# 0xMiden/miden-vm

Hardware: AMD Instinct MI355X
Metric: trace rows/sec proved (2^20-row trace, 96-bit sec) (higher is better)
Workload: dtype u64 (Goldilocks field, p = 2^64 - 2^32 + 1); 1 GPU; full proof of miden:20:51:8 (DummyMidenAir 2^20 x 51 + 8 EF aux), 96-bit production PCS params (blowup 8, FRI arity 4, 27 queries, PoW 4/12/16), Poseidon2 LMCS; trace resident in HBM, transcript on host; log_trace_rows=20, main_width=51, aux_width_ef=8, log_blowup=3, proof_bytes=137697, parallelism=1 GPU

## Files before the change

miden-vm_amd/csrc/deep.hip:

```cpp
#include "gl.cuh"
#include "kernels.hpp"

__global__ __launch_bounds__(256) void k_bary_weights(const u64* tw, int log_n, u64 g, e2 y0, e2 y1, u64* w0, u64* w1) {
  const size_t n = (size_t)1 << log_n;
  const size_t base = (size_t)blockIdx.x * 1024 + threadIdx.x;
  const size_t half = n >> 1;
  u64 xs[4], nrm[8], pre[8];
  e2 den[8];
#pragma unroll
  for (int k = 0; k < 4; k++) {
    size_t r = base + (size_t)k * 256;
    u64 x = 0;
    if (r < n) x = gl_mul(g, half ? (r < half ? tw[r] : gl_neg(tw[r - half])) : 1);
    xs[k] = x;
    den[2 * k] = e2_sub(y0, e2_make(x));
    den[2 * k + 1] = e2_sub(y1, e2_make(x));
  }
  u64 run = 1;
#pragma unroll
  for (int k = 0; k < 8; k++) {
    nrm[k] = gl_sub(gl_sqr(den[k].c0), gl_mul7(gl_sqr(den[k].c1)));
    pre[k] = run;
    run = gl_mul(run, nrm[k]);
  }
  u64 inv = gl_inv(run);
#pragma unroll
  for (int k = 7; k >= 0; k--) {
    u64 ni = gl_mul(inv, pre[k]);
    inv = gl_mul(inv, nrm[k]);
    size_t r = base + (size_t)(k >> 1) * 256;
    if (r < n) {
      u64 s = gl_mul(ni, xs[k >> 1]);
      u64* w = (k & 1) ? w1 : w0;
      w[2 * r] = gl_mul(den[k].c0, s);
      w[2 * r + 1] = gl_mul(gl_neg(den[k].c1), s);
    }
  }
}

static constexpr int OOD_ROWS_PER_BLOCK = 8192;
__global__ __launch_bounds__(256) void k_ood_partial(const u64* lde, int log_n, int log_blowup, const u64* w0, const u64* w1,
                                                     u64* partial, unsigned chunks) {
  __shared__ u64 red[4][256];
  const size_t n = (size_t)1 << log_n;
  const size_t col = blockIdx.y, chunk = blockIdx.x;
  const u64* f = lde + ((col << log_blowup) << log_n);
  const size_t r0 = chunk * OOD_ROWS_PER_BLOCK;
  const size_t r1 = r0 + OOD_ROWS_PER_BLOCK < n ? r0 + OOD_ROWS_PER_BLOCK : n;
  e2 a0 = e2_make(0), a1 = e2_make(0);
  for (size_t r = r0 + threadIdx.x; r < r1; r += 256) {
    u64 v = f[r];
    a0 = e2_add(a0, e2_mulf(e2{w0[2 * r], w0[2 * r + 1]}, v));
    a1 = e2_add(a1, e2_mulf(e2{w1[2 * r], w1[2 * r + 1]}, v));
  }
  red[0][threadIdx.x] = a0.c0; red[1][threadIdx.x] = a0.c1; red[2][threadIdx.x] = a1.c0; red[3][threadIdx.x] = a1.c1;
  __syncthreads();
  for (int s = 128; s > 0; s >>= 1) {
    if ((int)threadIdx.x < s) {
#pragma unroll
      for (int k = 0; k < 4; k++) red[k][threadIdx.x] = gl_add(red[k][threadIdx.x], red[k][threadIdx.x + s]);
    }
    __syncthreads();
  }
  if (threadIdx.x < 4) partial[(col * chunks + chunk) * 4 + threadIdx.x] = red[threadIdx.x][0];
}

void deep_ood_eval_batch(mh_ctx* c, std::vector<OodJob>& jobs, int log_blowup) {
  struct Weights {
    int log_n;
    size_t coset0;
    e2 y0, y1;
    DevBuf w0, w1;
  };
  std::vector<std::unique_ptr<Weights>> weights;
  struct Slot {
    size_t off = 0, ncol = 0;
    unsigned chunks = 0;
  };
  std::vector<Slot> slots(jobs.size());
  size_t total = 0;
  for (size_t k = 0; k < jobs.size(); k++) {
    OodJob& j = jobs[k];
    const LdeMatrix& m = *j.m;
    if (j.col_end > m.width) j.col_end = m.width;
    j.out0.assign(m.width, e2_make(0));
    j.out1.assign(m.width, e2_make(0));
    if (j.col_begin >= j.col_end) continue;
    const size_t n = (size_t)1 << m.log_n;
    slots[k].ncol = j.col_end - j.col_begin;
    slots[k].chunks = (unsigned)((n + OOD_ROWS_PER_BLOCK - 1) / OOD_ROWS_PER_BLOCK);
    slots[k].off = total;
    total += slots[k].ncol * slots[k].chunks * 4;
  }
  if (!total) return;
  DevBuf partial(total * 8), one;
  for (size_t k = 0; k < jobs.size(); k++) {
    if (!slots[k].ncol) continue;
    const OodJob& j = jobs[k];
    const LdeMatrix& m = *j.m;
    const int log_n = m.log_n;
    const size_t n = (size_t)1 << log_n;
    const u64 g = gl_mul(gl_lde_shift(log_n + log_blowup), gl_pow(gl_two_adic_generator(log_n + log_blowup), m.coset0));
    const u64* tw = log_n ? c->twiddles(log_n, false) : nullptr;
    if (!tw) {
      if (!one.p) {
        one.alloc(8);
        u64 v = 1;
        c->h2d(one.p, &v, 8);
      }
      tw = one.u();
    }
    ProfScope ps(c, "deep_ood_eval", (double)n * 8.0 * slots[k].ncol + 64.0 * n);
    Weights* w = nullptr;
    for (auto& cand : weights)
      if (cand->log_n == log_n && cand->coset0 == m.coset0 && e2_eq(cand->y0, j.y0) && e2_eq(cand->y1, j.y1)) w = cand.get();
    if (!w) {
      weights.emplace_back(new Weights{log_n, m.coset0, j.y0, j.y1, DevBuf(n * 16), DevBuf(n * 16)});
      w = weights.back().get();
      MH_LAUNCH(k_bary_weights, dim3((unsigned)((n + 1023) / 1024)), dim3(256), 0, c->stream, tw, log_n, g, j.y0, j.y1, w->w0.u(), w->w1.u());
    }
    MH_LAUNCH(k_ood_partial, dim3(slots[k].chunks, (unsigned)slots[k].ncol), dim3(256), 0, c->stream,
              m.lde.u() + ((j.col_begin << m.log_cosets) << log_n), log_n, m.log_cosets, w->w0.u(), w->w1.u(), partial.u() + slots[k].off,
              slots[k].chunks);
  }
  std::vector<u64> host(total);
  c->d2h(host.data(), partial.p, total * 8);
  for (size_t k = 0; k < jobs.size(); k++) {
    if (!slots[k].ncol) continue;
    OodJob& j = jobs[k];
    const LdeMatrix& m = *j.m;
    const int log_n = m.log_n;
    const size_t n = (size_t)1 << log_n;
    const u64 g = gl_mul(gl_lde_shift(log_n + log_blowup), gl_pow(gl_two_adic_generator(log_n + log_blowup), m.coset0));
    const u64 g_inv = gl_inv(g), n_inv = gl_inv((u64)n % GL_P);
    const e2 s0 = e2_mulf(e2_sub(e2_exp_pow2(e2_mulf(j.y0, g_inv), log_n), e2_make(1)), n_inv);
    const e2 s1 = e2_mulf(e2_sub(e2_exp_pow2(e2_mulf(j.y1, g_inv), log_n), e2_make(1)), n_inv);
    for (size_t col = 0; col < slots[k].ncol; col++) {
      e2 a0 = e2_make(0), a1 = e2_make(0);
      for (unsigned ch = 0; ch < slots[k].chunks; ch++) {
        const u64* p = host.data() + slots[k].off + (col * slots[k].chunks + ch) * 4;
        a0 = e2_add(a0, e2{p[0], p[1]});
        a1 = e2_add(a1, e2{p[2], p[3]});
      }
      j.out0[j.col_begin + col] = e2_mul(a0, s0);
      j.out1[j.col_begin + col] = e2_mul(a1, s1);
    }
  }
}
void deep_ood_eval_matrix(mh_ctx* c, const LdeMatrix& m, int log_blowup, e2 y0, e2 y1, std::vector<e2>& out0, std::vector<e2>& out1,
                          size_t col_begin, size_t col_end) {
  std::vector<OodJob> jobs(1);
  jobs[0].m = &m; jobs[0].y0 = y0; jobs[0].y1 = y1; jobs[0].col_begin = col_begin; jobs[0].col_end = col_end;
  deep_ood_eval_batch(c, jobs, log_blowup);
  out0.swap(jobs[0].out0);
  out1.swap(jobs[0].out1);
}

static constexpr int DEEP_MAX_MATS = 128;
static constexpr unsigned DEEP_FLUSH = 128;
#ifndef DEEP_UNROLL
#define DEEP_UNROLL 2
#endif
#ifndef DEEP_PTS_N
#define DEEP_PTS_N 1
#endif
static constexpr int DEEP_PTS = DEEP_PTS_N;
struct DeepMat {
  const u64* lde;
  u32 width, coef_off;
  int log_n;
};
struct DeepArgs {
  DeepMat m[DEEP_MAX_MATS];
  int n_mats, log_n, log_blowup;
  const u64* negc;
  const u64* tw;
  const u64* coset_x;
  e2 z0, z1, fred0, fred1, beta;
  u64* out;
};

__global__ __launch_bounds__(256) void k_deep_assemble(DeepArgs a) {
  const size_t N = (size_t)1 << a.log_n;
  const size_t j = blockIdx.y;
  const size_t base = (size_t)blockIdx.x * (256 * DEEP_PTS) + threadIdx.x;
  size_t r[DEEP_PTS];
#pragma unroll
  for (int k = 0; k < DEEP_PTS; k++) r[k] = base + (size_t)k * 256;
  e2 neg[DEEP_PTS];
  u64 w[DEEP_PTS][2][6];
#pragma unroll
  for (int k = 0; k < DEEP_PTS; k++) {
    neg[k] = e2_make(0);
#pragma unroll
    for (int e = 0; e < 2; e++)
#pragma unroll
      for (int i = 0; i < 6; i++) w[k][e][i] = 0;
  }
  auto flush = [&]() {
    const u64 C[6] = {1ULL, 1ULL << 22, 1ULL << 44, 1ULL << 32, 1ULL << 54, GL_EPS << 12};
#pragma unroll
    for (int k = 0; k < DEEP_PTS; k++) {
      u64 s0 = w[k][0][0], s1 = w[k][1][0];
#pragma unroll
      for (int i = 1; i < 6; i++) {
        s0 = gl_add(s0, gl_mul(w[k][0][i], C[i]));
        s1 = gl_add(s1, gl_mul(w[k][1][i], C[i]));
      }
      neg[k] = e2_add(neg[k], e2{s0, s1});
#pragma unroll
      for (int e = 0; e < 2; e++)
#pragma unroll
        for (int i = 0; i < 6; i++) w[k][e][i] = 0;
    }
  };
  u32 pending = 0;
#pragma unroll 1
  for (int mi = 0; mi < a.n_mats; mi++) {
    const DeepMat m = a.m[mi];
    const size_t nm_mask = ((size_t)1 << m.log_n) - 1;
    const u64* colp = m.lde + (j << m.log_n);
    const size_t cstride = (size_t)1 << (m.log_n + a.log_blowup);
#pragma unroll DEEP_UNROLL
    for (u32 cidx = 0; cidx < m.width; cidx++) {
      const u64 cf0 = a.negc[2 * (m.coef_off + cidx)], cf1 = a.negc[2 * (m.coef_off + cidx) + 1];
      u32 al[2][3];
#pragma unroll
      for (int i = 0; i < 3; i++) {
        al[0][i] = (u32)(cf0 >> (22 * i)) & 0x3FFFFFu;
        al[1][i] = (u32)(cf1 >> (22 * i)) & 0x3FFFFFu;
      }
#pragma unroll
      for (int k = 0; k < DEEP_PTS; k++) {
        if (r[k] < N) {
          const u64 v = colp[r[k] & nm_mask];
          const u32 v0 = (u32)v, v1 = (u32)(v >> 32);
#pragma unroll
          for (int e = 0; e < 2; e++) {
            w[k][e][0] += (u64)al[e][0] * v0;
            w[k][e][1] += (u64)al[e][1] * v0;
            w[k][e][2] += (u64)al[e][2] * v0;
            w[k][e][3] += (u64)al[e][0] * v1;
            w[k][e][4] += (u64)al[e][1] * v1;
            w[k][e][5] += (u64)al[e][2] * v1;
          }
        }
      }
      colp += cstride;
      if (++pending == DEEP_FLUSH) {
        flush();
        pending = 0;
      }
    }
  }
  flush();
  const size_t half = N >> 1;
  const u64 cx = a.coset_x[j];
  e2 den[2 * DEEP_PTS];
  u64 nrm[2 * DEEP_PTS], pre[2 * DEEP_PTS];
#pragma unroll
  for (int k = 0; k < DEEP_PTS; k++) {
    u64 x = 0;
    if (r[k] < N) x = gl_mul(cx, half ? (r[k] < half ? a.tw[r[k]] : gl_neg(a.tw[r[k] - half])) : 1);
    den[2 * k] = e2_sub(a.z0, e2_make(x));
    den[2 * k + 1] = e2_sub(a.z1, e2_make(x));
  }
  u64 run = 1;
#pragma unroll
  for (int k = 0; k < 2 * DEEP_PTS; k++) {
    nrm[k] = gl_sub(gl_sqr(den[k].c0), gl_mul7(gl_sqr(den[k].c1)));
    pre[k] = run;
    run = gl_mul(run, nrm[k]);
  }
  u64 inv = gl_inv(run);
  e2 qinv[2 * DEEP_PTS];
#pragma unroll
  for (int k = 2 * DEEP_PTS - 1; k >= 0; k--) {
    u64 ni = gl_mul(inv, pre[k]);
    inv = gl_mul(inv, nrm[k]);
    qinv[k] = e2{gl_mul(den[k].c0, ni), gl_mul(gl_neg(den[k].c1), ni)};
  }
#pragma unroll
  for (int k = 0; k < DEEP_PTS; k++) {
    if (r[k] < N) {
      e2 v = e2_mul(qinv[2 * k], e2_add(a.fred0, neg[k]));
      v = e2_add(v, e2_mul(e2_mul(a.beta, qinv[2 * k + 1]), e2_add(a.fred1, neg[k])));
      ulonglong2* o = reinterpret_cast<ulonglong2*>(a.out + 2 * ((j << a.log_n) + r[k]));
      *o = make_ulonglong2(v.c0, v.c1);
    }
  }
}

void deep_assemble(mh_ctx* c, const std::vector<const LdeMatrix*>& mats, const std::vector<u32>& coef_off, int log_n, int log_blowup,
                   const std::vector<e2>& negc, e2 z0, e2 z1, e2 fred0, e2 fred1, e2 beta, u64* out) {
  MH_REQUIRE(mats.size() <= (size_t)DEEP_MAX_MATS, "too many committed matrices for one DEEP pass");
  const int lbl = mats[0]->log_cosets;
  const size_t coset0 = mats[0]->coset0;
  for (auto* m : mats) MH_REQUIRE(m->log_cosets == lbl && m->coset0 == coset0, "internal: matrices cover different cosets");
  const size_t N = (size_t)1 << log_n, B = (size_t)1 << lbl;
  const int L = log_n + log_blowup;
  std::vector<u64> blob;
  for (e2 v : negc) { blob.push_back(v.c0); blob.push_back(v.c1); }
  const size_t o_cx = blob.size();
  const u64 g = gl_lde_shift(L), wK = gl_two_adic_generator(L);
  u64 x = gl_mul(g, gl_pow(wK, coset0));
  for (size_t j = 0; j < B; j++) {
    blob.push_back(x);
    x = gl_mul(x, wK);
  }
  DevBuf dblob(blob.size() * 8), one;
  c->h2d(dblob.p, blob.data(), blob.size() * 8);
  const u64* tw = log_n ? c->twiddles(log_n, false) : nullptr;
  if (!tw) {
    one.alloc(8);
    u64 v = 1;
    c->h2d(one.p, &v, 8);
    tw = one.u();
  }
  DeepArgs a{};
  double bytes = 16.0 * N * B;
  for (size_t i = 0; i < mats.size(); i++) {
    a.m[i] = DeepMat{mats[i]->lde.u(), (u32)mats[i]->width, coef_off[i], mats[i]->log_n};
    bytes += 8.0 * (double)mats[i]->width * (double)(((size_t)1 << mats[i]->log_n) << lbl);
  }
  a.n_mats = (int)mats.size();
  a.log_n = log_n; a.log_blowup = lbl;
  a.negc = dblob.u(); a.tw = tw; a.coset_x = dblob.u() + o_cx;
  a.z0 = z0; a.z1 = z1; a.fred0 = fred0; a.fred1 = fred1; a.beta = beta; a.out = out;
  {
    ProfScope ps(c, "deep_assemble", bytes);
    MH_LAUNCH(k_deep_assemble, dim3((unsigned)((N + 256 * DEEP_PTS - 1) / (256 * DEEP_PTS)), (unsigned)B), dim3(256), 0, c->stream, a);
  }
  HIP_CHECK(hipStreamSynchronize(c->stream));
}
```

miden-vm_amd/csrc/fri.hip:

```cpp
#include <cstring>
#include "gl.cuh"
#include "../../include/midenhip.h"
#include "kernels.hpp"
#include "blake3.cuh"
#include "keccak.cuh"
#include "poseidon2_fast.cuh"
#define RESCUE_FAST 1
#include "rescue.cuh"

__device__ __forceinline__ e2 ld_e2(const u64* p, size_t idx) {
  const ulonglong2 v = *reinterpret_cast<const ulonglong2*>(p + 2 * idx);
  return e2{v.x, v.y};
}
__device__ __forceinline__ void st_e2(u64* p, size_t idx, e2 v) { *reinterpret_cast<ulonglong2*>(p + 2 * idx) = make_ulonglong2(v.c0, v.c1); }

__device__ __forceinline__ u32 fri_row_pos(u32 p, int log_arity) { return bitrev32(p, log_arity); }

__global__ __launch_bounds__(256) void k_fri_leaf_hash(const u64* __restrict__ ev, int log_rows , int cbits, int log_arity,
                                                       u64* __restrict__ digests) {
  const int log_q = log_rows - log_arity;
  const size_t leaves = (size_t)1 << (log_q + cbits);
  const size_t s = blockIdx.x * (size_t)256 + threadIdx.x;
  if (s >= leaves) return;
  const size_t j = s >> log_q, r0 = s & (((size_t)1 << log_q) - 1);
  const u32 arity = 1u << log_arity;
  u64 st[12];
#pragma unroll
  for (int i = 0; i < 12; i++) st[i] = 0;
  for (u32 p0 = 0; p0 < arity; p0 += 4) {
#pragma unroll
    for (u32 k = 0; k < 4; k++) {
      e2 v = e2_make(0);
      if (p0 + k < arity) v = ld_e2(ev, (j << log_rows) + r0 + ((size_t)fri_row_pos(p0 + k, log_arity) << log_q));
      st[2 * k] = (p0 + k < arity) ? v.c0 : 0;
      st[2 * k + 1] = (p0 + k < arity) ? v.c1 : 0;
    }
    p2f_permute(st);
  }
  ulonglong2* o = reinterpret_cast<ulonglong2*>(digests + 4 * s);
  o[0] = make_ulonglong2(st[0], st[1]);
  o[1] = make_ulonglong2(st[2], st[3]);
}

__global__ __launch_bounds__(256) void k_fri_leaf_hash_b3(const u64* __restrict__ ev, int log_rows, int cbits, int log_arity,
                                                          u64* __restrict__ digests) {
  const int log_q = log_rows - log_arity;
  const size_t leaves = (size_t)1 << (log_q + cbits);
  const size_t s = blockIdx.x * (size_t)256 + threadIdx.x;
  if (s >= leaves) return;
  const size_t j = s >> log_q, r0 = s & (((size_t)1 << log_q) - 1);
  const u32 arity = 1u << log_arity;
  const u32 total = 32 + 16 * arity, n_blocks = (total + 63) / 64;
  b3::Stream h;
  h.init();
  uint32_t m[16], out[8];
#pragma unroll 1
  for (u32 b = 0; b < n_blocks; b++) {
    const int p0 = (int)(4 * b) - 2;
#pragma unroll
    for (int k = 0; k < 4; k++) {
      const int pp = p0 + k;
      e2 v = e2_make(0);
      if (pp >= 0 && (u32)pp < arity) v = ld_e2(ev, (j << log_rows) + r0 + ((size_t)fri_row_pos((u32)pp, log_arity) << log_q));
      m[4 * k] = (uint32_t)v.c0; m[4 * k + 1] = (uint32_t)(v.c0 >> 32);
      m[4 * k + 2] = (uint32_t)v.c1; m[4 * k + 3] = (uint32_t)(v.c1 >> 32);
    }
    if (b + 1 < n_blocks) h.block(m);
    else h.finish(m, total - 64 * b, out);
  }
#pragma unroll
  for (int i = 0; i < 4; i++) digests[4 * s + i] = (u64)out[2 * i] | ((u64)out[2 * i + 1] << 32);
}

__global__ __launch_bounds__(256) void k_fri_leaf_hash_alg(const u64* __restrict__ ev, int log_rows, int cbits, int log_arity,
                                                           u64* __restrict__ digests, int lmcs) {
  const int log_q = log_rows - log_arity;
  const size_t leaves = (size_t)1 << (log_q + cbits);
  const size_t s = blockIdx.x * (size_t)256 + threadIdx.x;
  if (s >= leaves) return;
  const size_t j = s >> log_q, r0 = s & (((size_t)1 << log_q) - 1);
  const u32 arity = 1u << log_arity;
  u64 st[12];
#pragma unroll
  for (int i = 0; i < 12; i++) st[i] = 0;
#pragma unroll 1
  for (u32 p0 = 0; p0 < arity; p0 += 4) {
#pragma unroll
    for (u32 k = 0; k < 4; k++) {
      e2 v = e2_make(0);
      if (p0 + k < arity) v = ld_e2(ev, (j << log_rows) + r0 + ((size_t)fri_row_pos(p0 + k, log_arity) << log_q));
      st[2 * k] = (p0 + k < arity) ? v.c0 : 0;
      st[2 * k + 1] = (p0 + k < arity) ? v.c1 : 0;
    }
    alg_permute(lmcs, st);
  }
#pragma unroll
  for (int i = 0; i < 4; i++) digests[4 * s + i] = st[i];
}

__global__ __launch_bounds__(256) void k_fri_leaf_hash_kk(const u64* __restrict__ ev, int log_rows, int cbits, int log_arity,
                                                          u64* __restrict__ digests) {
  const int log_q = log_rows - log_arity;
  const size_t leaves = (size_t)1 << (log_q + cbits);
  const size_t s = blockIdx.x * (size_t)256 + threadIdx.x;
  if (s >= leaves) return;
  const size_t j = s >> log_q, r0 = s & (((size_t)1 << log_q) - 1);
  const u32 arity = 1u << log_arity;
  uint64_t st[25];
#pragma unroll
  for (int i = 0; i < 25; i++) st[i] = 0;
#pragma unroll
  for (u32 p = 0; p < 8; p++) {
    if (p < arity) {
      const e2 v = ld_e2(ev, (j << log_rows) + r0 + ((size_t)fri_row_pos(p, log_arity) << log_q));
      st[2 * p] = v.c0;
      st[2 * p + 1] = v.c1;
    }
  }
  kk::f1600(st);
#pragma unroll
  for (int i = 0; i < 4; i++) digests[4 * s + i] = st[i];
}

struct FoldArgs {
  const u64* ev;
  u64* out;
  int log_rows, cbits, log_arity;
  const u64* tw_inv;
  const u64* coset_inv;
  e2 beta;
  u64 w4, w8_inv, inv_arity;
};
__global__ __launch_bounds__(256) void k_fri_fold(FoldArgs a) {
  const int log_q = a.log_rows - a.log_arity;
  const size_t total = (size_t)1 << (log_q + a.cbits);
  const size_t s = blockIdx.x * (size_t)256 + threadIdx.x;
  if (s >= total) return;
  const size_t j = s >> log_q, r0 = s & (((size_t)1 << log_q) - 1);
  const u64 s_inv = gl_mul(a.log_rows ? a.tw_inv[r0] : 1, a.coset_inv[j]);
  const e2 x = e2_mulf(a.beta, s_inv);
  const size_t base = (j << a.log_rows) + r0;
  e2 res;
  if (a.log_arity == 1) {
    e2 y0 = ld_e2(a.ev, base), y1 = ld_e2(a.ev, base + ((size_t)1 << log_q));
    res = e2_add(e2_add(y0, y1), e2_mul(e2_sub(y0, y1), x));
  } else if (a.log_arity == 3) {
    e2 y[8];
#pragma unroll
    for (int m = 0; m < 8; m++) y[m] = ld_e2(a.ev, base + ((size_t)m << log_q));
    const u64 wi1 = a.w8_inv, wi2 = gl_mul(wi1, wi1), wi3 = gl_mul(wi2, wi1);
#pragma unroll
    for (int m = 0; m < 4; m++) {
      const e2 u = y[m], v = y[m + 4];
      y[m] = e2_add(u, v);
      const e2 d = e2_sub(u, v);
      y[m + 4] = m == 0 ? d : e2_mulf(d, m == 1 ? wi1 : (m == 2 ? wi2 : wi3));
    }
#pragma unroll
    for (int h = 0; h < 8; h += 4)
#pragma unroll
      for (int m = 0; m < 2; m++) {
        const e2 u = y[h + m], v = y[h + m + 2];
        y[h + m] = e2_add(u, v);
        const e2 d = e2_sub(u, v);
        y[h + m + 2] = m == 0 ? d : e2_mulf(d, wi2);
      }
#pragma unroll
    for (int h = 0; h < 8; h += 2) {
      const e2 u = y[h], v = y[h + 1];
      y[h] = e2_add(u, v);
      y[h + 1] = e2_sub(u, v);
    }
    res = y[7];
    res = e2_add(e2_mul(res, x), y[3]);
    res = e2_add(e2_mul(res, x), y[5]);
    res = e2_add(e2_mul(res, x), y[1]);
    res = e2_add(e2_mul(res, x), y[6]);
    res = e2_add(e2_mul(res, x), y[2]);
    res = e2_add(e2_mul(res, x), y[4]);
    res = e2_add(e2_mul(res, x), y[0]);
  } else {
    e2 y0 = ld_e2(a.ev, base), y1 = ld_e2(a.ev, base + ((size_t)1 << log_q)), y2 = ld_e2(a.ev, base + ((size_t)2 << log_q)),
       y3 = ld_e2(a.ev, base + ((size_t)3 << log_q));
    e2 s02 = e2_add(y0, y2), d02 = e2_sub(y0, y2), s13 = e2_add(y1, y3), d31w = e2_mulf(e2_sub(y3, y1), a.w4);
    e2 c0 = e2_add(s02, s13), c1 = e2_add(d02, d31w), c2 = e2_sub(s02, s13), c3 = e2_sub(d02, d31w);
    e2 x2 = e2_sqr(x), x3 = e2_mul(x2, x);
    res = e2_add(e2_add(c0, e2_mul(c1, x)), e2_add(e2_mul(c2, x2), e2_mul(c3, x3)));
  }
  st_e2(a.out, s, e2_mulf(res, a.inv_arity));
}

__global__ void k_fri_to_natural(const u64* ev, u64* out, int log_rows, int cbits) {
  const size_t total = (size_t)1 << (log_rows + cbits);
  const size_t i = blockIdx.x * (size_t)blockDim.x + threadIdx.x;
  if (i >= total) return;
  const size_t j = i & (((size_t)1 << cbits) - 1), r = i >> cbits;
  st_e2(out, i, ld_e2(ev, (j << log_rows) + r));
}

void fri_leaf_hash(mh_ctx* c, const u64* ev, int log_rows, int cbits, int log_arity, u64* digests) {
  const size_t leaves = (size_t)1 << (log_rows - log_arity + cbits);
  ProfScope ps(c, "fri_leaf_hash", (double)leaves * (16.0 * (1 << log_arity) + 32.0));
  if (c->lmcs == MH_LMCS_RPO || c->lmcs == MH_LMCS_RPX)
    MH_LAUNCH(k_fri_leaf_hash_alg, dim3((unsigned)((leaves + 255) / 256)), dim3(256), 0, c->stream, ev, log_rows, cbits, log_arity, digests,
                       c->lmcs);
  else if (c->lmcs == MH_LMCS_KECCAK)
    MH_LAUNCH(k_fri_leaf_hash_kk, dim3((unsigned)((leaves + 255) / 256)), dim3(256), 0, c->stream, ev, log_rows, cbits, log_arity, digests);
  else if (c->lmcs == MH_LMCS_BLAKE3)
    MH_LAUNCH(k_fri_leaf_hash_b3, dim3((unsigned)((leaves + 255) / 256)), dim3(256), 0, c->stream, ev, log_rows, cbits, log_arity, digests);
  else
    MH_LAUNCH(k_fri_leaf_hash, dim3((unsigned)((leaves + 255) / 256)), dim3(256), 0, c->stream, ev, log_rows, cbits, log_arity,
                       digests);
}

void fri_fold(mh_ctx* c, const u64* ev, int log_rows, int cbits, int cbits_global, size_t coset0, int log_arity, e2 beta, u64* out) {
  MH_REQUIRE(log_arity >= 1 && log_arity <= 3, "FRI folding arity must be 2, 4 or 8");
  MH_REQUIRE(log_rows >= log_arity, "internal: FRI layer too short for a coset-major fold");
  const int logn = log_rows + cbits_global;
  const size_t C = (size_t)1 << cbits;
  std::vector<u64> ci(C);
  const u64 wn_inv = gl_inv(gl_two_adic_generator(logn));
  u64 x = gl_pow(wn_inv, coset0);
  for (size_t j = 0; j < C; j++) {
    ci[j] = x;
    x = gl_mul(x, wn_inv);
  }
  DevBuf d(C * 8);
  c->h2d(d.p, ci.data(), C * 8);
  FoldArgs a{};
  a.ev = ev; a.out = out; a.log_rows = log_rows; a.cbits = cbits; a.log_arity = log_arity;
  a.tw_inv = log_rows ? c->twiddles(log_rows, true) : nullptr;
  a.coset_inv = d.u();
  a.beta = beta;
  a.w4 = gl_two_adic_generator(2);
  a.w8_inv = gl_inv(gl_two_adic_generator(3));
  a.inv_arity = gl_inv((u64)1 << log_arity);
  const size_t total = (size_t)1 << (log_rows + cbits - log_arity);
  {
    ProfScope ps(c, "fri_fold", (double)total * 16.0 * ((1 << log_arity) + 1));
    MH_LAUNCH(k_fri_fold, dim3((unsigned)((total + 255) / 256)), dim3(256), 0, c->stream, a);
  }
  HIP_CHECK(hipStreamSynchronize(c->stream));
}

void fri_to_natural(mh_ctx* c, const u64* ev, int log_rows, int cbits, u64* out) {
  const size_t total = (size_t)1 << (log_rows + cbits);
  MH_LAUNCH(k_fri_to_natural, dim3((unsigned)((total + 255) / 256)), dim3(256), 0, c->stream, ev, out, log_rows, cbits);
}

struct GrindArgs {
  u64 st[12];
  u64 in[8];
  int n_in, bits;
  u64 base;
  unsigned long long* best;
};
__global__ __launch_bounds__(256) void k_grind(GrindArgs a) {
  const u64 w = a.base + blockIdx.x * (u64)256 + threadIdx.x;
  if (w >= GL_P) return;
  u64 s[12];
#pragma unroll
  for (int i = 0; i < 12; i++) s[i] = a.st[i];
  const int k = a.n_in + 1;
#pragma unroll
  for (int i = 0; i < 8; i++) {
    u64 v = (i < a.n_in) ? a.in[i] : (i == a.n_in ? w : 0);
    s[i] = (i < k) ? v : 0;
  }
  s[8] = gl_add(s[8], (u64)k);
  p2f_permute(s);
  const u64 x = s[7];
  if (((x & 0xFFFFFFFFULL) & (((u64)1 << a.bits) - 1)) == 0) atomicMin(a.best, (unsigned long long)w);
}

__global__ __launch_bounds__(256) void k_grind_alg(GrindArgs a, int lmcs) {
  const u64 w = a.base + blockIdx.x * (u64)256 + threadIdx.x;
  if (w >= GL_P) return;
  u64 s[12];
#pragma unroll
  for (int i = 0; i < 12; i++) s[i] = a.st[i];
  const int k = a.n_in + 1;
#pragma unroll
  for (int i = 0; i < 8; i++) {
    u64 v = (i < a.n_in) ? a.in[i] : (i == a.n_in ? w : 0);
    s[i] = (i < k) ? v : 0;
  }
  s[8] = gl_add(s[8], (u64)k);
  alg_permute(lmcs, s);
  if (((s[7] & 0xFFFFFFFFULL) & (((u64)1 << a.bits) - 1)) == 0) atomicMin(a.best, (unsigned long long)w);
}

struct GrindB3Args {
  b3::Stream pre;
  uint8_t tail[64];
  uint32_t tail_len;
  int bits;
  u64 base;
  unsigned long long* best;
};
__global__ __launch_bounds__(256) void k_grind_b3(GrindB3Args a) {
  const u64 w = a.base + blockIdx.x * (u64)256 + threadIdx.x;
  if (w >= GL_P) return;
  uint8_t buf[128];
#pragma unroll 1
  for (int i = 0; i < 128; i++) buf[i] = 0;
  for (uint32_t i = 0; i < a.tail_len; i++) buf[i] = a.tail[i];
  for (int k = 0; k < 8; k++) buf[a.tail_len + k] = (uint8_t)(w >> (8 * k));
  const uint32_t n = a.tail_len + 8;
  b3::Stream h = a.pre;
  uint32_t m[16], out[8];
  auto words = [&](const uint8_t* p) {
    for (int i = 0; i < 16; i++) m[i] = (uint32_t)p[4 * i] | ((uint32_t)p[4 * i + 1] << 8) | ((uint32_t)p[4 * i + 2] << 16) | ((uint32_t)p[4 * i + 3] << 24);
  };
  if (n <= 64) {
    words(buf);
    h.finish(m, n, out);
  } else {
    words(buf);
    h.block(m);
    words(buf + 64);
    h.finish(m, n - 64, out);
  }
  const u64 x = (u64)out[6] | ((u64)out[7] << 32);
  const u64 v = __builtin_bswap64(x);
  if ((v & (((u64)1 << a.bits) - 1)) == 0) atomicMin(a.best, (unsigned long long)w);
}
struct GrindKkArgs {
  u64 st[25];
  uint8_t tail[136];
  uint32_t tail_len;
  int bits;
  u64 base;
  unsigned long long* best;
};
__global__ __launch_bounds__(256) void k_grind_kk(GrindKkArgs a) {
  const u64 w = a.base + blockIdx.x * (u64)256 + threadIdx.x;
  if (w >= GL_P) return;
  kk::Sponge256 s;
  for (int i = 0; i < 25; i++) s.st[i] = a.st[i];
  for (uint32_t i = 0; i < a.tail_len; i++) s.buf[i] = a.tail[i];
  s.fill = a.tail_len;
  uint8_t wb[8], d[32];
  for (int k = 0; k < 8; k++) wb[k] = (uint8_t)(w >> (8 * k));
  s.update(wb, 8);
  s.finish(0x01, d);
  u64 v = 0;
  for (int i = 0; i < 8; i++) v |= (u64)d[31 - i] << (8 * i);
  if ((v & (((u64)1 << a.bits) - 1)) == 0) atomicMin(a.best, (unsigned long long)w);
}
u64 fri_grind_bytes(mh_ctx* c, int lmcs, const std::vector<uint8_t>& prefix, int bits) {
  MH_REQUIRE(bits > 0 && bits <= 32 && (lmcs == MH_LMCS_BLAKE3 || lmcs == MH_LMCS_KECCAK), "bad byte-challenger grind request");
  DevBuf best(8);
  GrindB3Args ab{};
  GrindKkArgs ak{};
  if (lmcs == MH_LMCS_BLAKE3) {
    MH_REQUIRE(prefix.size() + 8 <= ((size_t)1024 << b3::MAX_STACK) - 1024,
               "Blake3 PoW search: more than 255 KiB observed since the last sample (device stream stack)");
    ab.pre.init();
    const size_t k = prefix.size() / 64;
    for (size_t b = 0; b < k; b++) {
      uint32_t m[16];
      for (int i = 0; i < 16; i++) {
        const uint8_t* p = prefix.data() + 64 * b + 4 * i;
        m[i] = (uint32_t)p[0] | ((uint32_t)p[1] << 8) | ((uint32_t)p[2] << 16) | ((uint32_t)p[3] << 24);
      }
      ab.pre.block(m);
    }
    ab.tail_len = (uint32_t)(prefix.size() - 64 * k);
    memcpy(ab.tail, prefix.data() + 64 * k, ab.tail_len);
    ab.bits = bits;
    ab.best = (unsigned long long*)best.p;
  } else {
    kk::Sponge256 s;
    s.init();
    const size_t k = prefix.size() / 136;
    s.update(prefix.data(), 136 * k);
    for (int i = 0; i < 25; i++) ak.st[i] = s.st[i];
    ak.tail_len = (uint32_t)(prefix.size() - 136 * k);
    memcpy(ak.tail, prefix.data() + 136 * k, ak.tail_len);
    ak.bits = bits;
    ak.best = (unsigned long long*)best.p;
  }
  u64 window = (u64)1 << (bits + 2);
  if (window < 65536) window = 65536;
  ProfScope ps(c, "grind", 0);
  for (u64 base = 0;; base += window) {
    unsigned long long init = ~0ULL;
    c->h2d(best.p, &init, 8);
    if (lmcs == MH_LMCS_BLAKE3) {
      ab.base = base;
      MH_LAUNCH(k_grind_b3, dim3((unsigned)(window / 256)), dim3(256), 0, c->stream, ab);
    } else {
      ak.base = base;
      MH_LAUNCH(k_grind_kk, dim3((unsigned)(window / 256)), dim3(256), 0, c->stream, ak);
    }
    unsigned long long got = 0;
    c->d2h(&got, best.p, 8);
    if (got != ~0ULL) return (u64)got;
  }
}

u64 fri_grind(mh_ctx* c, const u64 st[12], const u64* in, int n_in, int bits) {
  MH_REQUIRE(bits > 0 && bits <= 32 && n_in >= 0 && n_in < 8, "bad grind request");
  DevBuf best(8);
  GrindArgs a{};
  for (int i = 0; i < 12; i++) a.st[i] = st[i];
  for (int i = 0; i < n_in; i++) a.in[i] = in[i];
  a.n_in = n_in; a.bits = bits;
  a.best = (unsigned long long*)best.p;
  u64 window = (u64)1 << (bits + 2);
  if (window < 65536) window = 65536;
  ProfScope ps(c, "grind", 0);
  for (u64 base = 0;; base += window) {
    unsigned long long init = ~0ULL;
    c->h2d(best.p, &init, 8);
    a.base = base;
    if (c->lmcs == MH_LMCS_RPO || c->lmcs == MH_LMCS_RPX)
      MH_LAUNCH(k_grind_alg, dim3((unsigned)(window / 256)), dim3(256), 0, c->stream, a, c->lmcs);
    else
      MH_LAUNCH(k_grind, dim3((unsigned)(window / 256)), dim3(256), 0, c->stream, a);
    unsigned long long got = 0;
    c->d2h(&got, best.p, 8);
    if (got != ~0ULL) return (u64)got;
  }
}
```

Baseline: 23.19 million trace rows/s.

## Drop stream syncs, inline fold coset constants, add lane-parallel Poseidon2 leaf hash

Removes the blocking stream synchronizations after DEEP assembly and each FRI fold, so the host keeps queuing work. Small FRI folds now pass their coset-inverse constants inside the kernel argument struct instead of allocating a device buffer and copying to it. For arity-4 FRI layers with few leaves, a new kernel hashes each leaf with 16 cooperating lanes using a lane-parallel Poseidon2 permutation, which improves occupancy on the small tail layers. The risks are hidden ordering dependencies on the removed syncs, and the DevBuf freed while the kernel may still be running is now avoided only when the inline path is taken.

```diff
diff --git a/miden-vm_amd/csrc/deep.hip b/miden-vm_amd/csrc/deep.hip
--- a/miden-vm_amd/csrc/deep.hip
+++ b/miden-vm_amd/csrc/deep.hip
@@ -331,5 +331,4 @@
     ProfScope ps(c, "deep_assemble", bytes);
     MH_LAUNCH(k_deep_assemble, dim3((unsigned)((N + 256 * DEEP_PTS - 1) / (256 * DEEP_PTS)), (unsigned)B), dim3(256), 0, c->stream, a);
   }
-  HIP_CHECK(hipStreamSynchronize(c->stream));
-}
+}
diff --git a/miden-vm_amd/csrc/fri.hip b/miden-vm_amd/csrc/fri.hip
--- a/miden-vm_amd/csrc/fri.hip
+++ b/miden-vm_amd/csrc/fri.hip
@@ -1,3 +1,4 @@
+#include <cstdlib>
 #include <cstring>
 #include "gl.cuh"
 #include "../../include/midenhip.h"
@@ -5,6 +6,7 @@
 #include "blake3.cuh"
 #include "keccak.cuh"
 #include "poseidon2_fast.cuh"
+#include "poseidon2_lanes.cuh"
 #define RESCUE_FAST 1
 #include "rescue.cuh"
 
@@ -40,6 +42,27 @@
   ulonglong2* o = reinterpret_cast<ulonglong2*>(digests + 4 * s);
   o[0] = make_ulonglong2(st[0], st[1]);
   o[1] = make_ulonglong2(st[2], st[3]);
+}
+
+static size_t fri_leaf_lanes_max_leaves() {
+  static const size_t v = [] {
+    const char* e = getenv("MH_FRI_LEAF_LANES_MAX");
+    return e ? (size_t)atol(e) : (size_t)8192;
+  }();
+  return v;
+}
+__global__ __launch_bounds__(256) void k_fri_leaf_hash_lanes(const u64* __restrict__ ev, int log_rows, int cbits, u64* __restrict__ digests) {
+  const int log_q = log_rows - 2;
+  const size_t leaves = (size_t)1 << (log_q + cbits);
+  const size_t leaf = (blockIdx.x * (size_t)256 + threadIdx.x) >> 4;
+  const int g = threadIdx.x & 15;
+  const bool active = leaf < leaves;
+  const size_t s = active ? leaf : 0;
+  const size_t j = s >> log_q, r0 = s & (((size_t)1 << log_q) - 1);
+  const size_t idx = (j << log_rows) + r0 + ((size_t)fri_row_pos((u32)(g >> 1) & 3, 2) << log_q);
+  u64 v = g < 8 ? ev[2 * idx + (g & 1)] : 0;
+  v = p2l_permute(v);
+  if (active && g < 4) digests[4 * s + g] = v;
 }
 
 __global__ __launch_bounds__(256) void k_fri_leaf_hash_b3(const u64* __restrict__ ev, int log_rows, int cbits, int log_arity,
@@ -122,12 +145,14 @@
   for (int i = 0; i < 4; i++) digests[4 * s + i] = st[i];
 }
 
+static constexpr int FOLD_COSETS_INLINE = 16;
 struct FoldArgs {
   const u64* ev;
   u64* out;
   int log_rows, cbits, log_arity;
   const u64* tw_inv;
   const u64* coset_inv;
+  u64 coset_inv_val[FOLD_COSETS_INLINE];
   e2 beta;
   u64 w4, w8_inv, inv_arity;
 };
@@ -137,7 +162,7 @@
   const size_t s = blockIdx.x * (size_t)256 + threadIdx.x;
   if (s >= total) return;
   const size_t j = s >> log_q, r0 = s & (((size_t)1 << log_q) - 1);
-  const u64 s_inv = gl_mul(a.log_rows ? a.tw_inv[r0] : 1, a.coset_inv[j]);
+  const u64 s_inv = gl_mul(a.log_rows ? a.tw_inv[r0] : 1, a.coset_inv ? a.coset_inv[j] : a.coset_inv_val[j]);
   const e2 x = e2_mulf(a.beta, s_inv);
   const size_t base = (j << a.log_rows) + r0;
   e2 res;
@@ -208,6 +233,8 @@
     MH_LAUNCH(k_fri_leaf_hash_kk, dim3((unsigned)((leaves + 255) / 256)), dim3(256), 0, c->stream, ev, log_rows, cbits, log_arity, digests);
   else if (c->lmcs == MH_LMCS_BLAKE3)
     MH_LAUNCH(k_fri_leaf_hash_b3, dim3((unsigned)((leaves + 255) / 256)), dim3(256), 0, c->stream, ev, log_rows, cbits, log_arity, digests);
+  else if (log_arity == 2 && leaves <= fri_leaf_lanes_max_leaves())
+    MH_LAUNCH(k_fri_leaf_hash_lanes, dim3((unsigned)((leaves * 16 + 255) / 256)), dim3(256), 0, c->stream, ev, log_rows, cbits, digests);
   else
     MH_LAUNCH(k_fri_leaf_hash, dim3((unsigned)((leaves + 255) / 256)), dim3(256), 0, c->stream, ev, log_rows, cbits, log_arity,
                        digests);
@@ -218,6 +245,7 @@
   MH_REQUIRE(log_rows >= log_arity, "internal: FRI layer too short for a coset-major fold");
   const int logn = log_rows + cbits_global;
   const size_t C = (size_t)1 << cbits;
+  FoldArgs a{};
   std::vector<u64> ci(C);
   const u64 wn_inv = gl_inv(gl_two_adic_generator(logn));
   u64 x = gl_pow(wn_inv, coset0);
@@ -225,9 +253,13 @@
     ci[j] = x;
     x = gl_mul(x, wn_inv);
   }
-  DevBuf d(C * 8);
-  c->h2d(d.p, ci.data(), C * 8);
-  FoldArgs a{};
+  DevBuf d;
+  if (C <= (size_t)FOLD_COSETS_INLINE) {
+    memcpy(a.coset_inv_val, ci.data(), C * 8);
+  } else {
+    d.alloc(C * 8);
+    c->h2d(d.p, ci.data(), C * 8);
+  }
   a.ev = ev; a.out = out; a.log_rows = log_rows; a.cbits = cbits; a.log_arity = log_arity;
   a.tw_inv = log_rows ? c->twiddles(log_rows, true) : nullptr;
   a.coset_inv = d.u();
@@ -240,7 +272,6 @@
     ProfScope ps(c, "fri_fold", (double)total * 16.0 * ((1 << log_arity) + 1));
     MH_LAUNCH(k_fri_fold, dim3((unsigned)((total + 255) / 256)), dim3(256), 0, c->stream, a);
   }
-  HIP_CHECK(hipStreamSynchronize(c->stream));
 }
 
 void fri_to_natural(mh_ctx* c, const u64* ev, int log_rows, int cbits, u64* out) {
```

Measured after the change: 23.39 million trace rows/s (median of 6 runs). About the same (+0.9%).
